# Superjomn/TiPS

Measured on AMD Instinct MI355X. Metric: device-resident fp32 bucket-sum GiB/s (% HBM peak); allreduce GiB/s 1/2/4/8 GPU, higher is better.
Workload: dtype f32

## Files before the change

### tips_amd/csrc/fusion.cc

```cpp
#include <string.h>

#include <algorithm>

#include "rt.h"

namespace tips {
namespace rt {

namespace {

constexpr int64_t kDefaultCopyTile = 8 * 1024;
constexpr size_t kMaxLayouts = 32;
constexpr size_t kMaxTables = 16;
constexpr int kUploadSlots = 4;

int64_t copy_tile_bytes() {
  const int64_t t = env_i64("TIPS_COPY_TILE_BYTES", kDefaultCopyTile);
  return t <= 4096 ? 4096 : t <= 8192 ? 8192 : 16384;
}

int64_t cast_tile_bytes() {
  const int64_t t = env_i64("TIPS_CAST_TILE_BYTES", 4096);
  return t <= 4096 ? 4096 : t <= 8192 ? 8192 : 16384;
}
// ... 264 lines not shown
      const size_t share = std::min<size_t>((size_t)cap, (slow.size() - si + (7 - x)) / (8 - x));
      for (size_t k = 0; k < share; k++) xcd[x].push_back(slow[si++]);
    }
    for (int x = 0; x < 8; x++) {
      const int cap = std::max(0, std::min(R, n - x * R));
      while ((int)xcd[x].size() < cap && si < slow.size()) xcd[x].push_back(slow[si++]);
      while ((int)xcd[x].size() < cap && fi < fast.size()) xcd[x].push_back(fast[fi++]);
    }
    int at = g0;
    for (int x = 0; x < 8; x++)
      for (int j : xcd[x]) order[at++] = j;
  }
  return order;
}

void fill_records(const Layout& L, int mode, const BatchItem* items, const void* base, std::vector<CopySeg>* dst) {
  const int nseg = (int)L.seg_tensor.size();
  const int ntab = tables_of(mode);
  const size_t per = 2 * (size_t)L.ntiles + nseg;
  const int64_t es = tips::dtype_size(L.dtype);
  std::vector<CopySeg>& rec = *dst;
  rec.assign(ntab * per, CopySeg{0, 0, 0, 0});
  for (int k = 0; k < nseg; k++) {
    const int i = L.seg_tensor[k];
    const int64_t b = L.off[i], e = b + L.counts[i] * es;
    const int64_t in = (int64_t)(uintptr_t)items[i].in - b, out = (int64_t)(uintptr_t)items[i].out - b;
    CopySeg* r = rec.data() + 2 * L.ntiles + k;
    if (mode == kSlot || mode == kSlotCast) {
      const int bk = L.bucket[i];
      const int64_t slot = bk < 0 ? 0 : (int64_t)(uintptr_t)base + (int64_t)(bk % 2) * L.threshold - L.buckets[bk].off;
      const int64_t win = (int64_t)(uintptr_t)items[i].in - 2 * b, wout = (int64_t)(uintptr_t)items[i].out - 2 * b;
// ... 4 lines not shown
    } else {
      r[0] = CopySeg{in, (int64_t)(uintptr_t)base, b, e};
    }
  }
  const std::vector<int> order = tile_order(L);
  for (int tb = 0; tb < ntab; tb++) {
    CopySeg* T = rec.data() + tb * per;
    const CopySeg* S = T + 2 * L.ntiles;
    for (int q = 0; q < L.ntiles; q++) {
      const int j = order[q];
      const int first = L.tiles[2 * j], cnt = L.tiles[2 * j + 1];
      T[2 * q] = cnt <= 2 ? S[first] : CopySeg{first, cnt, 0, -1};
      T[2 * q + 1] = cnt == 2 ? S[first + 1] : CopySeg{0, 0, (int64_t)j * L.tile, 0};
    }
  }
}

Table* find_table(State& st, FusionCache& fc, Layout& L, int mode, const BatchItem* items, int n,
                  const void* base) {
  uint64_t h = fnv(fnv(kFnvBasis, (uint64_t)mode), (uint64_t)(uintptr_t)base);
  for (int i = 0; i < n; i++) h = fnv(fnv(h, (uint64_t)(uintptr_t)items[i].in), (uint64_t)(uintptr_t)items[i].out);
  for (Table* t : L.tables) {
    if (t->hash != h || t->mode != mode || t->base != base) continue;
    bool same = true;
    for (int i = 0; i < n && same; i++) same = t->ins[i] == items[i].in && t->outs[i] == items[i].out;
    if (same) {
      t->stamp = ++fc.clock;
      fc.table_hits++;
      if (st.fuse_capturing) t->pinned = true;
      return t;
// ... 6 lines not shown
  }
  Table* t = nullptr;
  size_t unpinned = 0;
  for (const Table* u : L.tables) unpinned += !u->pinned;
  if (unpinned >= kMaxTables) {
    auto lru = L.tables.end();
    for (auto it = L.tables.begin(); it != L.tables.end(); ++it)
      if (!(*it)->pinned && (lru == L.tables.end() || (*it)->stamp < (*lru)->stamp)) lru = it;
    if ((*lru)->mode == mode) {
      t = *lru;
    } else {
      free_table(st, *lru);
      L.tables.erase(lru);
    }
  }
  const int nseg = (int)L.seg_tensor.size();
  const int ntab = tables_of(mode);
  const size_t per = 2 * (size_t)L.ntiles + nseg;
  if (!t) {
    t = new Table();
    if (hipMallocAsync((void**)&t->dev, ntab * per * sizeof(CopySeg), table_stream(st)) != hipSuccess) {
      delete t;
      fail(TIPS_ERR_HIP, "fusion: hipMallocAsync of a segment table failed");
      return nullptr;
    }
    L.tables.push_back(t);
  }
  t->hash = h;
  t->mode = mode;
  t->base = base;
  t->ins.resize(n);
  t->outs.resize(n);
  for (int i = 0; i < n; i++) {
    t->ins[i] = items[i].in;
    t->outs[i] = items[i].out;
  }
  std::vector<CopySeg> rec;
  fill_records(L, mode, items, base, &rec);
  t->stamp = ++fc.clock;
  fc.tables_built++;
  if (upload(st, fc, t->dev, rec.data(), rec.size() * sizeof(CopySeg)) != 0 ||
      (st.fuse_in_call && join(st.fuse_ws, st.fuse_stream, st.ev_fuse_table) != 0)) {
    t->hash = 0;
    t->ins.clear();
    return nullptr;
  }
  return t;
}

int ensure_slots(State& st, FusionCache& fc, int64_t threshold) {
  if (threshold == st.fusion_threshold && st.fusion.p) return 0;
  bool pinned = false;
  for (const Layout* L : fc.layouts) pinned = pinned || L->pinned();
  if (st.fuse_chain_valid) {
    TRY(chain_event(st));
    HIP_TRY(hipEventSynchronize(st.ev_fuse_chain));
// ... 26 lines not shown
}

int open_layout(State& st, FusionCache& fc, const BatchItem* items, int n, int dtype, const LayoutParams& lp,
                hipStream_t ws, Layout** L) {
  if (st.size > 1) {
    HIP_TRY(hipEventRecord(st.ev_start, ws));
    HIP_TRY(hipStreamWaitEvent(st.bucket_stream, st.ev_start, 0));
  }
  std::vector<int64_t> counts((size_t)n);
  for (int i = 0; i < n; i++) counts[i] = items[i].count;
  *L = find_layout(st, fc, counts.data(), n, dtype, lp);
  return 0;
}

struct Records {
  const CopySeg *tiles, *segs;
};
Records records(const Layout& L, const Table& t, int table) {
  const CopySeg* base = t.dev + (size_t)table * (2 * (size_t)L.ntiles + L.seg_tensor.size());
  return {base, base + 2 * L.ntiles};
}

int copy_tiles(const Layout& L, const Table& t, int table, int tile0, int ntiles, hipStream_t s) {
  const Records r = records(L, t, table);
  HIP_TRY(tips::launch_copy_segs(r.tiles, r.segs, tile0, ntiles, L.tile, copy_store_policy(), s));
  return 0;
}

bool pack_merge(const State& st) { return !st.fuse_capturing && env_i64("TIPS_PACK_MERGE", 0) != 0; }

bool pack_signals_ready(State& st, hipStream_t ws) {
  if (st.pack_signals >= 0) return st.pack_signals == 1;
  st.pack_signals = 0;
  if (env_i64("TIPS_PACK_SIGNALS", 1) == 0) return false;
  int can = 0;
  if (hipDeviceGetAttribute(&can, hipDeviceAttributeCanUseStreamWaitValue, st.device) != hipSuccess || !can) {
    (void)hipGetLastError();
    return false;
  }
  bool ok = hipMalloc((void**)&st.pack_counters, tips::kMaxPackGroups * sizeof(unsigned)) == hipSuccess &&
// ... 14 lines not shown

int pack_buckets(State& st, const Layout& L, const Table& t, int table, int b0, int nb, bool signal, uint64_t* values,
                 hipStream_t s) {
  tips::PackGroups g{};
  g.n = nb;
  g.counters = signal ? st.pack_counters : nullptr;
  for (int k = 0; k < nb; k++) {
    g.tile0[k] = L.buckets[b0 + k].tile0;
    g.ntiles[k] = L.buckets[b0 + k].ntiles;
    if (signal) {
      g.done[k] = static_cast<unsigned long long*>(st.pack_done[k]);
      g.sig_value[k] = st.pack_done_value[k] + 1;
    }
  }
  const Records r = records(L, t, table);
  HIP_TRY(tips::launch_copy_segs_groups(r.tiles, r.segs, g, L.tile, copy_store_policy(), s));
  if (signal)
    for (int k = 0; k < nb; k++) values[k] = ++st.pack_done_value[k];
  return 0;
}

int wait_packed(State& st, int k, uint64_t value) {
  HIP_TRY(hipStreamWaitValue64(st.bucket_stream, st.pack_done[k], value, hipStreamWaitValueGte, ~0ull));
  return 0;
}

struct MergedPacks {
  std::function<int(int)> pack;
  std::function<int(int, hipEvent_t)> wait;
};

// ... 258 lines not shown
  if (n <= 0) return 0;
  FusionCache& fc = cache(st);
  const LayoutParams lp = layout_params(true);
  TRY(ensure_slots(st, fc, lp.threshold));
  return in_fusion(st, user, [&](hipStream_t ws) -> int {
    Layout* L = nullptr;
    TRY(open_layout(st, fc, items, n, wire, lp, ws, &L));
    if (!L) return TIPS_ERR_HIP;
    if (L->seg_tensor.empty()) return 0;
    const int64_t es = tips::dtype_size(wire);
    const int B = (int)L->buckets.size();
    Table* t = B ? find_table(st, fc, *L, kSlotCast, items, n, st.fusion.p) : nullptr;
    if (B && !t) return TIPS_ERR_HIP;
    auto cast = [&](int dir, int b) -> int {
      const Records r = records(*L, *t, dir);
      HIP_TRY(tips::launch_cast_segs(r.tiles, r.segs, L->buckets[b].tile0, L->buckets[b].ntiles, L->tile, dir, wire, ws));
      return 0;
    };
    hipStream_t big = st.size > 1 ? st.bucket_stream : ws;
    for (int i : L->direct) {
      TRY(st.cast_scratch.ensure((size_t)(items[i].count * es)));
      HIP_TRY(tips::launch_cast_range(st.cast_scratch.p, items[i].in, items[i].count, 0, wire, big));
      if (st.size > 1) TRY(allreduce_device(st, st.cast_scratch.p, st.cast_scratch.p, items[i].count, wire, big));
      HIP_TRY(tips::launch_cast_range(items[i].out, st.cast_scratch.p, items[i].count, 1, wire, big));
    }
    if (st.size == 1) {
      for (int b = 0; b < B; b++) {
        TRY(cast(0, b));
        TRY(cast(1, b));
      }
      return 0;
// ... 61 lines not shown
  if (dtype != TIPS_FLOAT32)
    return fail(TIPS_ERR_UNSUPPORTED, "tips_fused_allreduce_cast: the tensors must be TIPS_FLOAT32 (got dtype %d)", dtype);
  if (wire_dtype != TIPS_FLOAT16 && wire_dtype != TIPS_BFLOAT16)
    return fail(TIPS_ERR_UNSUPPORTED, "tips_fused_allreduce_cast: the wire type must be TIPS_FLOAT16 or TIPS_BFLOAT16 "
                                      "(got %d)", wire_dtype);
  if (!outs && n > 0) return fail(TIPS_ERR_INVALID_ARG, "bad tensor list");
  return list_collective(ins, counts, n, dtype, wire_dtype, kOutsEach, outs, nullptr, true,
                         [&](State& st, std::vector<BatchItem>& items) {
                           return fused_allreduce_cast(st, items.data(), n, wire_dtype, (hipStream_t)stream);
                         });
}

#ifdef TIPS_DEV
int64_t tips_fusion_tile_table(const int64_t* counts, int n, int dtype, const int64_t* ins, const int64_t* outs,
                               int64_t* records, int64_t cap, int64_t* ntiles, int64_t* tile_bytes) {
  TRY(check_dtype(dtype));
  if (n < 0 || (n > 0 && (!counts || !ins || !outs))) return fail(TIPS_ERR_INVALID_ARG, "bad list");
  for (int i = 0; i < n; i++)
    if (counts[i] < 0) return fail(TIPS_ERR_INVALID_ARG, "negative count %d", i);
  Layout L;
  build_layout(&L, dtype, layout_params(), counts, n);
  std::vector<BatchItem> items((size_t)n);
  for (int i = 0; i < n; i++) items[i] = BatchItem{(const void*)(uintptr_t)ins[i], (void*)(uintptr_t)outs[i], counts[i]};
  std::vector<tips::CopySeg> rec;
  fill_records(L, kCopy, items.data(), nullptr, &rec);
  if (ntiles) *ntiles = L.ntiles;
  if (tile_bytes) *tile_bytes = L.tile;
  if (records) {
    if (cap < (int64_t)rec.size()) return fail(TIPS_ERR_INVALID_ARG, "tips_fusion_tile_table: %zu records, room for %lld", rec.size(), (long long)cap);
    memcpy(records, rec.data(), rec.size() * sizeof(tips::CopySeg));
  }
  return (int64_t)rec.size();
}
#endif

int64_t tips_fused_layout(const int64_t* counts, int n, int dtype, int64_t* offsets) {
  TRY(check_dtype(dtype));
  if (n < 0 || (n > 0 && !counts)) return fail(TIPS_ERR_INVALID_ARG, "bad count list");
  for (int i = 0; i < n; i++)
    if (counts[i] < 0) return fail(TIPS_ERR_INVALID_ARG, "negative count %d", i);
// ... 70 lines not shown
```

### tips_amd/csrc/kernels.h

```cpp
#pragma once

#include <hip/hip_runtime.h>
#include <stdint.h>

#include <vector>

namespace tips {

int dtype_size(int dtype);

hipError_t launch_sum2(void* dst, const void* a, const void* b, int64_t n, int dtype, hipStream_t s);

constexpr int kMaxSrcs = 16;
hipError_t launch_multi_sum(void* dst, const void* const* srcs, int nsrc, int64_t n, int dtype, hipStream_t s);
hipError_t launch_multi_sum_remote(void* dst, const void* const* srcs, int nsrc, int64_t n, int dtype, hipStream_t s);

enum { kOpSum = 0, kOpMax = 1, kOpMin = 2 };
hipError_t launch_reduce2(void* dst, const void* a, const void* b, int64_t n, int dtype, int op, hipStream_t s);
hipError_t launch_multi_reduce(void* dst, const void* const* srcs, int nsrc, int64_t n, int dtype, int op, hipStream_t s);

struct Scale {
  double pre = 1.0, post = 1.0;
  int op = kOpSum;
  bool on() const { return pre != 1.0 || post != 1.0; }
  bool minmax() const { return op != kOpSum; }
  bool plain() const { return !on() && !minmax(); }
};
hipError_t launch_sum2_scaled(void* dst, const void* a, const void* b, int64_t n, int dtype, double pre, double post,
                              unsigned raw, hipStream_t s);
hipError_t launch_multi_sum_scaled(void* dst, const void* const* srcs, int nsrc, int64_t n, int dtype, double pre,
                                   double post, unsigned raw, hipStream_t s);
hipError_t launch_scale_buf(void* dst, const void* src, int64_t n, int dtype, double pre, double post, hipStream_t s);

struct CopySeg {
  int64_t src, dst;
  int64_t begin, end;
};
hipError_t launch_copy_segs(const CopySeg* tiles, const CopySeg* segs, int tile0, int ntiles, int64_t tile_bytes,
                            int pol, hipStream_t s);
int64_t pack_stripe_vecs();
void stripe_slots(int64_t nslots, int64_t C, std::vector<int>* xcd, std::vector<int64_t>* pos);

constexpr int kMaxPackGroups = 8;
struct PackGroups {
  int n;
  int tile0[kMaxPackGroups], ntiles[kMaxPackGroups];
  unsigned blk0[kMaxPackGroups + 1];
  unsigned* counters;
  unsigned long long* done[kMaxPackGroups];
  unsigned long long sig_value[kMaxPackGroups];
};
hipError_t launch_copy_segs_groups(const CopySeg* tiles, const CopySeg* segs, PackGroups g, int64_t tile_bytes, int pol,
                                   hipStream_t s);

hipError_t launch_cast_segs(const CopySeg* tiles, const CopySeg* segs, int tile0, int ntiles, int64_t tile_bytes,
                            int dir, int wire, hipStream_t s);
hipError_t launch_cast_range(void* dst, const void* src, int64_t n, int dir, int wire, hipStream_t s);

hipError_t launch_copy_buf(void* dst, const void* src, int64_t bytes, hipStream_t s);

struct XferSeg {
  const char* src;
  char* dst;
  int64_t bytes;
};
constexpr int kMaxXferSegs = 16;
constexpr int64_t kXferTileBytes = 16 * 1024;
hipError_t launch_xfer(const XferSeg* segs, int nseg, hipStream_t s);

}
```

### tips_amd/csrc/kernels.hip

```cpp
#include <algorithm>
#include <cstdlib>
#include <type_traits>

#include "kernels_device.h"

namespace tips {

int dtype_size(int dtype) {
  switch (dtype) {
    case kF32: return 4;
    case kF64: return 8;
    case kI32: return 4;
    case kI64: return 8;
    case kF16: return 2;
    case kBF16: return 2;
    default: return 0;
  }
}

typedef __attribute__((address_space(1))) u32x4 g_u32x4;
typedef __attribute__((address_space(1))) unsigned g_u32;
typedef __attribute__((address_space(1))) unsigned short g_u16;
typedef __attribute__((address_space(1))) char g_u8;

// ... 39 lines not shown
#pragma unroll
    for (int k = 0; k < 4; k++)
      if (4 * k < len) *reinterpret_cast<g_u32*>(d + 4 * k) = m.w[k];
  } else {
#pragma unroll
    for (int k = 0; k < 8; k++)
      if (2 * k < len) *reinterpret_cast<g_u16*>(d + 2 * k) = m.h[k];
  }
}

template <int U>
struct SegStage {
  CopySeg L[(int)((int64_t)kBlock * 16 * U / 256) + 1];
};

template <int U, int POL>
__device__ __forceinline__ void copy_seg_tile(const CopySeg* __restrict__ tiles, const CopySeg* __restrict__ segs,
                                              int t, CopySeg* L) {
  constexpr int64_t kTileBytes = (int64_t)kBlock * 16 * U;
  constexpr int kMaxSeg = (int)(kTileBytes / 256) + 1;
  const int64_t* tr = reinterpret_cast<const int64_t*>(tiles + 2 * (int64_t)t);
  const int64_t a_src = tr[0], a_dst = tr[1], a_beg = tr[2], a_end = tr[3];
  const int64_t b_src = tr[4], b_dst = tr[5], b_beg = tr[6], b_end = tr[7];
  const int tid = threadIdx.x;
  const bool multi = a_end < 0, two = b_end > 0;
  const int64_t tb = two ? (b_beg & ~(kTileBytes - 1)) : b_beg;
  if (!multi && !two && a_beg <= tb && a_end >= tb + kTileBytes && ((a_src | a_dst) & 15) == 0) {
    __amdgpu_buffer_rsrc_t rs = __builtin_amdgcn_make_buffer_rsrc((void*)(a_src + tb), (short)0, (int)kTileBytes,
                                                                  0x00020000);
    __amdgpu_buffer_rsrc_t rd = __builtin_amdgcn_make_buffer_rsrc((void*)(a_dst + tb), (short)0, (int)kTileBytes,
                                                                  0x00020000);
    u32x4 v[U];
#pragma unroll
    for (int u = 0; u < U; u++) v[u] = __builtin_amdgcn_raw_buffer_load_b128(rs, (u * kBlock + tid) * 16, 0, 2);
#pragma unroll
    for (int u = 0; u < U; u++)
      __builtin_amdgcn_raw_buffer_store_b128(v[u], rd, (u * kBlock + tid) * 16, 0, POL == 0 ? 0 : POL == 1 ? 2 : 16);
    return;
  }
  int cnt = 1;
  if (multi) {
    const int s0 = (int)a_src;
    cnt = min((int)a_dst, kMaxSeg);
    if (cnt <= 0) return;
    if (tid < cnt) L[tid] = segs[s0 + tid];
    __syncthreads();
  }
  int64_t sp[U], dp[U];
  int len[U];
  bool full[U];
  u32x4 x[U];
  Small m[U];
#pragma unroll
  for (int u = 0; u < U; u++) {
// ... 21 lines not shown
    len[u] = (v >= g_beg && left > 0) ? (int)(left < 16 ? left : 16) : 0;
    sp[u] = g_src + v;
    dp[u] = g_dst + v;
    full[u] = len[u] == 16 && ((sp[u] | dp[u]) & 15) == 0;
    if (full[u]) x[u] = __builtin_nontemporal_load(reinterpret_cast<const g_u32x4*>(sp[u]));
    else if (len[u] > 0) small_load(sp[u], dp[u], len[u], m[u]);
  }
#pragma unroll
  for (int u = 0; u < U; u++) {
    if (full[u]) store16_pol<POL>(dp[u], x[u]);
    else if (len[u] > 0) small_store(sp[u], dp[u], len[u], m[u]);
  }
}

template <int U, int POL>
__global__ __launch_bounds__(kBlock) void copy_segs_kernel(const CopySeg* __restrict__ tiles,
                                                          const CopySeg* __restrict__ segs, int tile0, int ntiles,
                                                          int64_t stripe) {
  __shared__ SegStage<U> st;
  const int64_t tt = stripe_tile(blockIdx.x, gridDim.x, stripe);
  if (tt >= ntiles) return;
  copy_seg_tile<U, POL>(tiles, segs, tile0 + (int)tt, st.L);
}


template <int WT>
__device__ __forceinline__ u32x2 narrow4(f32x4 a) {
  if constexpr (WT == kF16) {
    return __builtin_bit_cast(u32x2, __builtin_convertvector(a, f16x4));
  } else {
    const u32x4 x = __builtin_bit_cast(u32x4, a);
    return u32x2{bf16_round_bits(x[0]) | (bf16_round_bits(x[1]) << 16), bf16_round_bits(x[2]) | (bf16_round_bits(x[3]) << 16)};
  }
}

template <int WT>
__device__ __forceinline__ f32x4 widen4(u32x2 v) {
// ... 33 lines not shown
  } else {
    u32x4 x[U];
#pragma unroll
    for (int u = 0; u < U; u++)
      x[u] = __builtin_nontemporal_load(reinterpret_cast<const g_u32x4*>(wire_base + 16 * (int64_t)(u * kBlock + tid)));
#pragma unroll
    for (int u = 0; u < U; u++) reinterpret_cast<u32x4*>(W)[u * kBlock + tid] = x[u];
    __syncthreads();
#pragma unroll
    for (int u = 0; u < 2 * U; u++)
      store16_pol<2>(f32_base + 16 * (int64_t)(u * kBlock + tid), __builtin_bit_cast(u32x4, widen4<WT>(W[u * kBlock + tid])));
  }
}

template <int U, int DIR, int WT, int VAR = 8>
__global__ __launch_bounds__(kBlock) void cast_segs_kernel(const CopySeg* __restrict__ tiles,
                                                          const CopySeg* __restrict__ segs, int tile0, int ntiles) {
  constexpr int64_t kTileBytes = (int64_t)kBlock * 16 * U;
  constexpr int kMaxSeg = (int)(kTileBytes / 256) + 1;
  constexpr int Q = 2 * U;
  __shared__ CopySeg L[kMaxSeg];
  const int64_t tt = xcd_tile(blockIdx.x, gridDim.x);
  if (tt >= ntiles) return;
  const int64_t* tr = reinterpret_cast<const int64_t*>(tiles + 2 * (int64_t)(tile0 + tt));
  const int64_t a_src = tr[0], a_dst = tr[1], a_beg = tr[2], a_end = tr[3];
  const int64_t b_src = tr[4], b_dst = tr[5], b_beg = tr[6], b_end = tr[7];
  const int tid = threadIdx.x;
  const bool multi = a_end < 0, two = b_end > 0;
  const int64_t tb = two ? (b_beg & ~(kTileBytes - 1)) : b_beg;
  if constexpr ((VAR & 8) != 0) {
    __shared__ u32x2 W[kBlock * Q];
    if (!multi && !two && a_beg <= tb && a_end >= tb + kTileBytes && ((a_src | a_dst) & 15) == 0) {
      if constexpr (DIR == 0) cast_tile_staged<U, 0, WT>(a_src + 2 * tb, a_dst + tb, W);
      else cast_tile_staged<U, 1, WT>(a_dst + 2 * tb, a_src + tb, W);
      return;
    }
  }
  int cnt = 1;
  if (multi) {
    cnt = min((int)a_dst, kMaxSeg);
    if (cnt <= 0) return;
    if (tid < cnt) L[tid] = segs[(int)a_src + tid];
    __syncthreads();
  }
  int64_t sp[Q], dp[Q];
  int len[Q];
  bool full[Q];
  u32x2 nv[Q];
  f32x4 wa[Q];
#pragma unroll
  for (int u = 0; u < Q; u++) {
    const int64_t v = tb + (int64_t)u * (kBlock * 8) + (int64_t)tid * 8;
// ... 75 lines not shown
      if constexpr (DIR == 0)
        store8_sc1(wire_side + 8 * q, narrow4<WT>(__builtin_nontemporal_load(reinterpret_cast<const g_f32x4*>(f32_side + 16 * q))));
      else
        store16_pol<2>(f32_side + 16 * q, __builtin_bit_cast(u32x4, widen4<WT>(
                                              __builtin_nontemporal_load(reinterpret_cast<const g_u32x2*>(wire_side + 8 * q)))));
    }
    head = 4 * nq;
  }
  for (int64_t i = head + (int64_t)blockIdx.x * kBlock + threadIdx.x; i < n; i += stride) {
    if constexpr (DIR == 0) static_cast<unsigned short*>(dst)[i] = narrow1<WT>(static_cast<const float*>(src)[i]);
    else static_cast<float*>(dst)[i] = widen1<WT>(static_cast<const unsigned short*>(src)[i]);
  }
}

template <int U, int POL>
__global__ __launch_bounds__(kBlock) void copy_segs_groups_kernel(const CopySeg* __restrict__ tiles,
                                                                 const CopySeg* __restrict__ segs, PackGroups g) {
  __shared__ SegStage<U> st;
  int k = 0;
  while (k + 1 < g.n && blockIdx.x >= g.blk0[k + 1]) k++;
  const unsigned local = blockIdx.x - g.blk0[k], gk = g.blk0[k + 1] - g.blk0[k];
  const int64_t tt = xcd_tile(local, gk);
  if (tt < g.ntiles[k]) copy_seg_tile<U, POL>(tiles, segs, g.tile0[k] + (int)tt, st.L);
  if (g.done[k]) {
    __syncthreads();
    if (threadIdx.x == 0 &&
        __hip_atomic_fetch_add(&g.counters[k], 1u, __ATOMIC_ACQ_REL, __HIP_MEMORY_SCOPE_AGENT) == gk - 1) {
      __hip_atomic_store(&g.counters[k], 0u, __ATOMIC_RELAXED, __HIP_MEMORY_SCOPE_AGENT);
      __hip_atomic_store(g.done[k], g.sig_value[k], __ATOMIC_RELEASE, __HIP_MEMORY_SCOPE_SYSTEM);
    }
  }
}


struct XferList {
  XferSeg s[kMaxXferSegs];
};

// ... 364 lines not shown
  if (nsrc == 1) return launch_multi_sum(dst, srcs, nsrc, n, dtype, s);
  switch (dtype) {
    case kF32: return multi_dispatch<kF32>(dst, srcs, nsrc, n, s, true);
    case kF64: return multi_dispatch<kF64>(dst, srcs, nsrc, n, s, true);
    case kI32: return multi_dispatch<kI32>(dst, srcs, nsrc, n, s, true);
    case kI64: return multi_dispatch<kI64>(dst, srcs, nsrc, n, s, true);
    case kF16: return multi_dispatch<kF16>(dst, srcs, nsrc, n, s, true);
    case kBF16: return multi_dispatch<kBF16>(dst, srcs, nsrc, n, s, true);
    default: return hipErrorInvalidValue;
  }
}

namespace {

template <int U>
hipError_t run_copy_segs_groups(const CopySeg* tiles, const CopySeg* segs, const PackGroups& g, int pol, hipStream_t s) {
  const unsigned grid = g.blk0[g.n];
  switch (pol) {
    case 0: hipLaunchKernelGGL((copy_segs_groups_kernel<U, 0>), dim3(grid), dim3(kBlock), 0, s, tiles, segs, g); break;
    case 1: hipLaunchKernelGGL((copy_segs_groups_kernel<U, 1>), dim3(grid), dim3(kBlock), 0, s, tiles, segs, g); break;
    case 2: hipLaunchKernelGGL((copy_segs_groups_kernel<U, 2>), dim3(grid), dim3(kBlock), 0, s, tiles, segs, g); break;
    default: return hipErrorInvalidValue;
  }
  return hipGetLastError();
}

template <int U>
hipError_t run_copy_segs(const CopySeg* tiles, const CopySeg* segs, int tile0, int ntiles, int pol, hipStream_t s) {
  const int64_t C = pack_stripe_vecs() / ((int64_t)kBlock * U);
  const unsigned grid = (unsigned)stripe_grid(ntiles, C);
  switch (pol) {
    case 0: hipLaunchKernelGGL((copy_segs_kernel<U, 0>), dim3(grid), dim3(kBlock), 0, s, tiles, segs, tile0, ntiles, C); break;
    case 1: hipLaunchKernelGGL((copy_segs_kernel<U, 1>), dim3(grid), dim3(kBlock), 0, s, tiles, segs, tile0, ntiles, C); break;
    case 2: hipLaunchKernelGGL((copy_segs_kernel<U, 2>), dim3(grid), dim3(kBlock), 0, s, tiles, segs, tile0, ntiles, C); break;
    default: return hipErrorInvalidValue;
  }
  return hipGetLastError();
}

}

hipError_t launch_copy_segs(const CopySeg* tiles, const CopySeg* segs, int tile0, int ntiles, int64_t tile_bytes,
                            int pol, hipStream_t s) {
  if (ntiles <= 0) return hipSuccess;
  switch (tile_bytes) {
    case 4096: return run_copy_segs<1>(tiles, segs, tile0, ntiles, pol, s);
    case 8192: return run_copy_segs<2>(tiles, segs, tile0, ntiles, pol, s);
    case 16384: return run_copy_segs<4>(tiles, segs, tile0, ntiles, pol, s);
    default: return hipErrorInvalidValue;
  }
}

hipError_t launch_copy_segs_groups(const CopySeg* tiles, const CopySeg* segs, PackGroups g, int64_t tile_bytes, int pol,
                                   hipStream_t s) {
  if (g.n < 1 || g.n > kMaxPackGroups) return hipErrorInvalidValue;
  for (int k = 0; k < g.n; k++)
    if (g.done[k] && !g.counters) return hipErrorInvalidValue;
  int64_t blk = 0;
  for (int k = 0; k < g.n; k++) {
    if (g.ntiles[k] < 0) return hipErrorInvalidValue;
    g.blk0[k] = (unsigned)blk;
    blk += std::max<int64_t>(8, ((int64_t)g.ntiles[k] + 7) / 8 * 8);
  }
  if (blk > 0x7fffffff) return hipErrorInvalidValue;
  g.blk0[g.n] = (unsigned)blk;
  switch (tile_bytes) {
    case 4096: return run_copy_segs_groups<1>(tiles, segs, g, pol, s);
    case 8192: return run_copy_segs_groups<2>(tiles, segs, g, pol, s);
    case 16384: return run_copy_segs_groups<4>(tiles, segs, g, pol, s);
    default: return hipErrorInvalidValue;
  }
}

namespace {
int cast_lds_bytes(int dir) {
  static const int v[2] = {(int)std::min<long>(65536, std::max<long>(0, getenv("TIPS_CAST_LDS_PACK") ? atol(getenv("TIPS_CAST_LDS_PACK")) : 0)),
                           (int)std::min<long>(65536, std::max<long>(0, getenv("TIPS_CAST_LDS_UNPACK") ? atol(getenv("TIPS_CAST_LDS_UNPACK")) : 0))};
  return v[dir];
}

template <int U, int DIR>
hipError_t run_cast_segs(const CopySeg* tiles, const CopySeg* segs, int tile0, int ntiles, int wire, hipStream_t s) {
  const unsigned grid = (unsigned)std::max<int64_t>(8, ((int64_t)ntiles + 7) / 8 * 8);
  const int lds = cast_lds_bytes(DIR);
  static const int var = getenv("TIPS_CAST_VARIANT") ? atoi(getenv("TIPS_CAST_VARIANT")) : 8;
  if (wire != kF16 && wire != kBF16) return hipErrorInvalidValue;
  auto kern = wire == kF16 ? &cast_segs_kernel<U, DIR, kF16> : &cast_segs_kernel<U, DIR, kBF16>;
  if constexpr (U == 2) {
    if (wire == kF16 && var != 8)
      kern = var == 0   ? &cast_segs_kernel<U, DIR, kF16, 0>
             : var == 1 ? &cast_segs_kernel<U, DIR, kF16, 1>
             : var == 2 ? &cast_segs_kernel<U, DIR, kF16, 2>
             : var == 3 ? &cast_segs_kernel<U, DIR, kF16, 3>
             : var == 4 ? &cast_segs_kernel<U, DIR, kF16, 4>
                        : &cast_segs_kernel<U, DIR, kF16, 5>;
  }
  hipLaunchKernelGGL(kern, dim3(grid), dim3(kBlock), lds, s, tiles, segs, tile0, ntiles);
  return hipGetLastError();
}

template <int DIR>
hipError_t run_cast_range(void* dst, const void* src, int64_t n, int wire, hipStream_t s) {
  const int64_t grid = std::max<int64_t>(1, std::min<int64_t>((n + kBlock - 1) / kBlock, (int64_t)kNumCUs * 16));
  if (wire == kF16) hipLaunchKernelGGL((cast_range_kernel<DIR, kF16>), dim3((unsigned)grid), dim3(kBlock), 0, s, dst, src, n);
  else if (wire == kBF16) hipLaunchKernelGGL((cast_range_kernel<DIR, kBF16>), dim3((unsigned)grid), dim3(kBlock), 0, s, dst, src, n);
  else return hipErrorInvalidValue;
  return hipGetLastError();
}
}

hipError_t launch_cast_segs(const CopySeg* tiles, const CopySeg* segs, int tile0, int ntiles, int64_t tile_bytes,
                            int dir, int wire, hipStream_t s) {
  if (ntiles <= 0) return hipSuccess;
  if (dir != 0 && dir != 1) return hipErrorInvalidValue;
  switch (tile_bytes) {
    case 4096: return dir ? run_cast_segs<1, 1>(tiles, segs, tile0, ntiles, wire, s) : run_cast_segs<1, 0>(tiles, segs, tile0, ntiles, wire, s);
    case 8192: return dir ? run_cast_segs<2, 1>(tiles, segs, tile0, ntiles, wire, s) : run_cast_segs<2, 0>(tiles, segs, tile0, ntiles, wire, s);
    case 16384: return dir ? run_cast_segs<4, 1>(tiles, segs, tile0, ntiles, wire, s) : run_cast_segs<4, 0>(tiles, segs, tile0, ntiles, wire, s);
    default: return hipErrorInvalidValue;
  }
}

hipError_t launch_cast_range(void* dst, const void* src, int64_t n, int dir, int wire, hipStream_t s) {
  if (n <= 0) return hipSuccess;
  return dir ? run_cast_range<1>(dst, src, n, wire, s) : run_cast_range<0>(dst, src, n, wire, s);
}

hipError_t launch_xfer(const XferSeg* segs, int nseg, hipStream_t s) {
  if (nseg < 0 || nseg > kMaxXferSegs) return hipErrorInvalidValue;
  XferList L{};
  int64_t max_tiles = 0;
  int m = 0;
  for (int i = 0; i < nseg; i++) {
// ... 14 lines not shown
```

### tips_amd/csrc/kernels_dev.hip

```cpp
#include <algorithm>

#include "kernels_dev.h"
#include "kernels_device.h"

namespace tips {

template <int DT, int MODE, int UNROLL, bool NTL, bool NTS, int BLOCK>
__global__ __launch_bounds__(BLOCK) void sum2_kernel(u32x4* __restrict__ dst, const u32x4* __restrict__ a,
                                                    const u32x4* __restrict__ b, int64_t nvec, int64_t tail_begin,
                                                    int64_t n) {
  constexpr int64_t kTile = (int64_t)BLOCK * UNROLL;
  const int tid = threadIdx.x;
  int64_t t = (MODE == 2) ? xcd_tile(blockIdx.x, gridDim.x) : (int64_t)blockIdx.x;
  const int64_t tstride = (MODE == 0) ? (int64_t)gridDim.x : 0;
  do {
    const int64_t base = t * kTile + tid;
    if (base + (UNROLL - 1) * BLOCK < nvec) {
      u32x4 x[UNROLL], y[UNROLL];
#pragma unroll
      for (int u = 0; u < UNROLL; u++) x[u] = ld16<NTL>(a + base + u * BLOCK);
#pragma unroll
      for (int u = 0; u < UNROLL; u++) y[u] = ld16<NTL>(b + base + u * BLOCK);
#pragma unroll
      for (int u = 0; u < UNROLL; u++) st16<NTS>(dst + base + u * BLOCK, add16<DT>(x[u], y[u]));
    } else {
#pragma unroll
      for (int u = 0; u < UNROLL; u++) {
        const int64_t i = base + u * BLOCK;
        if (i < nvec) st16<NTS>(dst + i, add16<DT>(ld16<NTL>(a + i), ld16<NTL>(b + i)));
      }
    }
    t += tstride;
  } while (MODE == 0 && t * kTile < nvec);
  if (blockIdx.x == 0 && tail_begin + tid < n) add_elem<DT>(dst, a, b, tail_begin + tid);
}

__global__ __launch_bounds__(256) void sum2_map_kernel(u32x4* __restrict__ dst, const u32x4* __restrict__ a,
                                                       const u32x4* __restrict__ b, int64_t nvec, int64_t tail_begin,
                                                       int64_t n, int64_t stripe) {
  constexpr int64_t kTile = 256;
  const int64_t bx = blockIdx.x, x = bx & 7, j = bx >> 3;
  const int64_t t = stripe == 0 ? bx : (x + 8 * (j / stripe)) * stripe + j % stripe;
  const int64_t first = t * kTile;
  if (first < nvec) {
    const int rec = (int)(((nvec - first) < kTile ? (nvec - first) : kTile) * 16);
    __amdgpu_buffer_rsrc_t ra = __builtin_amdgcn_make_buffer_rsrc((void*)(a + first), (short)0, rec, 0x00020000);
    __amdgpu_buffer_rsrc_t rb = __builtin_amdgcn_make_buffer_rsrc((void*)(b + first), (short)0, rec, 0x00020000);
    __amdgpu_buffer_rsrc_t rd = __builtin_amdgcn_make_buffer_rsrc((void*)(dst + first), (short)0, rec, 0x00020000);
    const u32x4 xv = __builtin_amdgcn_raw_buffer_load_b128(ra, (int)threadIdx.x * 16, 0, 2);
// ... 290 lines not shown

template <int DT>
hipError_t sum2_dispatch(void* dst, const void* a, const void* b, int64_t n, int mode, int unroll, int nt, int blocks,
                         int threads, hipStream_t s) {
  if (!(aligned16(dst) && aligned16(a) && aligned16(b))) return launch_sum2(dst, a, b, n, DT, s);
  if (mode == 5) {
    if constexpr (DT == kF32) {
      if (threads == 256 && (unroll == 1 || unroll == 2 || unroll == 4 || unroll == 8)) {
        const int64_t nvec = n / 4;
        hipLaunchKernelGGL(sum2_stream_kernel, dim3((unsigned)(kNumCUs * unroll)), dim3(256), 0, s, (u32x4*)dst,
                           (const u32x4*)a, (const u32x4*)b, nvec, nvec * 4, n);
        return hipGetLastError();
      }
    }
    return hipErrorInvalidValue;
  }
  if (mode == 6) {
    if constexpr (DT == kF32) {
      const int64_t nvec = n / 4, T = (nvec + 255) / 256;
      const int64_t stripe = (int64_t)unroll * 1024 / 4096;
      if (unroll < 0 || (unroll > 0 && stripe < 1)) return hipErrorInvalidValue;
      const int64_t grid = stripe == 0 ? std::max<int64_t>(1, T) : ((T + stripe - 1) / stripe + 7) / 8 * 8 * stripe;
      hipLaunchKernelGGL(sum2_map_kernel, dim3((unsigned)grid), dim3(256), 0, s, (u32x4*)dst, (const u32x4*)a,
                         (const u32x4*)b, nvec, nvec * 4, n, stripe);
      return hipGetLastError();
    }
    return hipErrorInvalidValue;
  }
  if (mode == 4) {
    if constexpr (DT == kF32) {
// ... 327 lines not shown
```

Before: 6296.

## Add precomputed per-tile descriptors for fast-path whole-tile copies and casts

Builds a compact per-tile descriptor table (absolute src/dst addresses) alongside the existing segment records. Kernels check it first and take the single-segment buffer copy or cast path without reading and decoding the 64-byte tile records. Descriptors are loaded into scalar registers, and a look-ahead touch warms the descriptor cache for later tiles. The change also adds a dev-only bound copy kernel mode. The cost is a larger device table, extra upload bytes, and one more dependent load on the slow path.

```diff
diff --git a/tips_amd/csrc/fusion.cc b/tips_amd/csrc/fusion.cc
--- a/tips_amd/csrc/fusion.cc
+++ b/tips_amd/csrc/fusion.cc
@@ -302,7 +302,8 @@
   return order;
 }
 
-void fill_records(const Layout& L, int mode, const BatchItem* items, const void* base, std::vector<CopySeg>* dst) {
+void fill_records(const Layout& L, int mode, const BatchItem* items, const void* base, std::vector<CopySeg>* dst,
+                  std::vector<tips::TileDesc>* descs) {
   const int nseg = (int)L.seg_tensor.size();
   const int ntab = tables_of(mode);
   const size_t per = 2 * (size_t)L.ntiles + nseg;
@@ -337,6 +338,24 @@
       T[2 * q + 1] = cnt == 2 ? S[first + 1] : CopySeg{0, 0, (int64_t)j * L.tile, 0};
     }
   }
+  descs->assign((size_t)ntab * L.ntiles, tips::TileDesc{tips::kDescRecords, 0});
+  for (int tb = 0; tb < ntab; tb++) {
+    const CopySeg* S = rec.data() + tb * per + 2 * L.ntiles;
+    const int64_t ks = mode == kSlotCast && tb == 0 ? 2 : 1, kd = mode == kSlotCast && tb == 1 ? 2 : 1;
+    for (int q = 0; q < L.ntiles; q++) {
+      const int j = order[q];
+      const int64_t v = (int64_t)j * L.tile;
+      if (L.tiles[2 * j + 1] != 1) continue;
+      const CopySeg& g = S[L.tiles[2 * j]];
+      if (g.begin <= v && g.end >= v + L.tile && ((g.src | g.dst) & 15) == 0)
+        (*descs)[(size_t)tb * L.ntiles + q] = tips::TileDesc{g.src + ks * v, g.dst + kd * v};
+    }
+  }
+}
+
+size_t table_bytes(const Layout& L, int mode) {
+  const size_t per = 2 * (size_t)L.ntiles + L.seg_tensor.size();
+  return tables_of(mode) * (per * sizeof(CopySeg) + (size_t)L.ntiles * sizeof(tips::TileDesc));
 }
 
 Table* find_table(State& st, FusionCache& fc, Layout& L, int mode, const BatchItem* items, int n,
@@ -373,12 +392,9 @@
       L.tables.erase(lru);
     }
   }
-  const int nseg = (int)L.seg_tensor.size();
-  const int ntab = tables_of(mode);
-  const size_t per = 2 * (size_t)L.ntiles + nseg;
   if (!t) {
     t = new Table();
-    if (hipMallocAsync((void**)&t->dev, ntab * per * sizeof(CopySeg), table_stream(st)) != hipSuccess) {
+    if (hipMallocAsync((void**)&t->dev, table_bytes(L, mode), table_stream(st)) != hipSuccess) {
       delete t;
       fail(TIPS_ERR_HIP, "fusion: hipMallocAsync of a segment table failed");
       return nullptr;
@@ -395,10 +411,14 @@
     t->outs[i] = items[i].out;
   }
   std::vector<CopySeg> rec;
-  fill_records(L, mode, items, base, &rec);
+  std::vector<tips::TileDesc> descs;
+  fill_records(L, mode, items, base, &rec, &descs);
+  const size_t nrec = rec.size();
+  rec.resize(nrec + (descs.size() + 1) / 2);
+  memcpy(static_cast<void*>(rec.data() + nrec), descs.data(), descs.size() * sizeof(tips::TileDesc));
   t->stamp = ++fc.clock;
   fc.tables_built++;
-  if (upload(st, fc, t->dev, rec.data(), rec.size() * sizeof(CopySeg)) != 0 ||
+  if (upload(st, fc, t->dev, rec.data(), table_bytes(L, mode)) != 0 ||
       (st.fuse_in_call && join(st.fuse_ws, st.fuse_stream, st.ev_fuse_table) != 0)) {
     t->hash = 0;
     t->ins.clear();
@@ -455,16 +475,19 @@
 }
 
 struct Records {
+  const tips::TileDesc* desc;
   const CopySeg *tiles, *segs;
 };
 Records records(const Layout& L, const Table& t, int table) {
-  const CopySeg* base = t.dev + (size_t)table * (2 * (size_t)L.ntiles + L.seg_tensor.size());
-  return {base, base + 2 * L.ntiles};
+  const size_t per = 2 * (size_t)L.ntiles + L.seg_tensor.size();
+  const CopySeg* base = t.dev + (size_t)table * per;
+  const tips::TileDesc* desc = reinterpret_cast<const tips::TileDesc*>(t.dev + (size_t)tables_of(t.mode) * per);
+  return {desc + (size_t)table * L.ntiles, base, base + 2 * L.ntiles};
 }
 
 int copy_tiles(const Layout& L, const Table& t, int table, int tile0, int ntiles, hipStream_t s) {
   const Records r = records(L, t, table);
-  HIP_TRY(tips::launch_copy_segs(r.tiles, r.segs, tile0, ntiles, L.tile, copy_store_policy(), s));
+  HIP_TRY(tips::launch_copy_segs(r.desc, r.tiles, r.segs, tile0, ntiles, L.tile, copy_store_policy(), s));
   return 0;
 }
 
@@ -509,7 +532,7 @@
     }
   }
   const Records r = records(L, t, table);
-  HIP_TRY(tips::launch_copy_segs_groups(r.tiles, r.segs, g, L.tile, copy_store_policy(), s));
+  HIP_TRY(tips::launch_copy_segs_groups(r.desc, r.tiles, r.segs, g, L.tile, copy_store_policy(), s));
   if (signal)
     for (int k = 0; k < nb; k++) values[k] = ++st.pack_done_value[k];
   return 0;
@@ -798,7 +821,7 @@
     if (B && !t) return TIPS_ERR_HIP;
     auto cast = [&](int dir, int b) -> int {
       const Records r = records(*L, *t, dir);
-      HIP_TRY(tips::launch_cast_segs(r.tiles, r.segs, L->buckets[b].tile0, L->buckets[b].ntiles, L->tile, dir, wire, ws));
+      HIP_TRY(tips::launch_cast_segs(r.desc, r.tiles, r.segs, L->buckets[b].tile0, L->buckets[b].ntiles, L->tile, dir, wire, ws));
       return 0;
     };
     hipStream_t big = st.size > 1 ? st.bucket_stream : ws;
@@ -890,16 +913,27 @@
 #ifdef TIPS_DEV
 int64_t tips_fusion_tile_table(const int64_t* counts, int n, int dtype, const int64_t* ins, const int64_t* outs,
                                int64_t* records, int64_t cap, int64_t* ntiles, int64_t* tile_bytes) {
+  constexpr uintptr_t kTestSlotBase = (uintptr_t)1 << 41;
   TRY(check_dtype(dtype));
   if (n < 0 || (n > 0 && (!counts || !ins || !outs))) return fail(TIPS_ERR_INVALID_ARG, "bad list");
   for (int i = 0; i < n; i++)
     if (counts[i] < 0) return fail(TIPS_ERR_INVALID_ARG, "negative count %d", i);
+  const int64_t with_descs = env_i64("TIPS_TILE_TABLE_DESCS", 0);
+  const bool cast = with_descs == 2;
+  if (cast && dtype != TIPS_FLOAT16 && dtype != TIPS_BFLOAT16)
+    return fail(TIPS_ERR_INVALID_ARG, "tips_fusion_tile_table: a cast table's dtype is the wire type (got %d)", dtype);
   Layout L;
-  build_layout(&L, dtype, layout_params(), counts, n);
+  build_layout(&L, dtype, layout_params(cast), counts, n);
   std::vector<BatchItem> items((size_t)n);
   for (int i = 0; i < n; i++) items[i] = BatchItem{(const void*)(uintptr_t)ins[i], (void*)(uintptr_t)outs[i], counts[i]};
   std::vector<tips::CopySeg> rec;
-  fill_records(L, kCopy, items.data(), nullptr, &rec);
+  std::vector<tips::TileDesc> descs;
+  fill_records(L, cast ? kSlotCast : kCopy, items.data(), cast ? (const void*)kTestSlotBase : nullptr, &rec, &descs);
+  if (with_descs != 0) {
+    const size_t nrec = rec.size();
+    rec.resize(nrec + (descs.size() + 1) / 2, tips::CopySeg{0, 0, 0, 0});
+    memcpy(static_cast<void*>(rec.data() + nrec), descs.data(), descs.size() * sizeof(tips::TileDesc));
+  }
   if (ntiles) *ntiles = L.ntiles;
   if (tile_bytes) *tile_bytes = L.tile;
   if (records) {
diff --git a/tips_amd/csrc/kernels.h b/tips_amd/csrc/kernels.h
--- a/tips_amd/csrc/kernels.h
+++ b/tips_amd/csrc/kernels.h
@@ -36,8 +36,12 @@
   int64_t src, dst;
   int64_t begin, end;
 };
-hipError_t launch_copy_segs(const CopySeg* tiles, const CopySeg* segs, int tile0, int ntiles, int64_t tile_bytes,
-                            int pol, hipStream_t s);
+struct TileDesc {
+  int64_t src, dst;
+};
+constexpr int64_t kDescRecords = 1;
+hipError_t launch_copy_segs(const TileDesc* desc, const CopySeg* tiles, const CopySeg* segs, int tile0, int ntiles,
+                            int64_t tile_bytes, int pol, hipStream_t s);
 int64_t pack_stripe_vecs();
 void stripe_slots(int64_t nslots, int64_t C, std::vector<int>* xcd, std::vector<int64_t>* pos);
 
@@ -50,11 +54,11 @@
   unsigned long long* done[kMaxPackGroups];
   unsigned long long sig_value[kMaxPackGroups];
 };
-hipError_t launch_copy_segs_groups(const CopySeg* tiles, const CopySeg* segs, PackGroups g, int64_t tile_bytes, int pol,
-                                   hipStream_t s);
+hipError_t launch_copy_segs_groups(const TileDesc* desc, const CopySeg* tiles, const CopySeg* segs, PackGroups g,
+                                   int64_t tile_bytes, int pol, hipStream_t s);
 
-hipError_t launch_cast_segs(const CopySeg* tiles, const CopySeg* segs, int tile0, int ntiles, int64_t tile_bytes,
-                            int dir, int wire, hipStream_t s);
+hipError_t launch_cast_segs(const TileDesc* desc, const CopySeg* tiles, const CopySeg* segs, int tile0, int ntiles,
+                            int64_t tile_bytes, int dir, int wire, hipStream_t s);
 hipError_t launch_cast_range(void* dst, const void* src, int64_t n, int dir, int wire, hipStream_t s);
 
 hipError_t launch_copy_buf(void* dst, const void* src, int64_t bytes, hipStream_t s);
diff --git a/tips_amd/csrc/kernels.hip b/tips_amd/csrc/kernels.hip
--- a/tips_amd/csrc/kernels.hip
+++ b/tips_amd/csrc/kernels.hip
@@ -77,30 +77,42 @@
   CopySeg L[(int)((int64_t)kBlock * 16 * U / 256) + 1];
 };
 
+__device__ __forceinline__ TileDesc load_desc(const TileDesc* __restrict__ desc, int64_t t) {
+  const int64_t* p = reinterpret_cast<const int64_t*>(desc + t);
+  TileDesc d{p[0], p[1]};
+  asm volatile("" : "+s"(d.src), "+s"(d.dst));
+  return d;
+}
+
+constexpr int kAheadSlots = 32 * 8;
+__device__ __forceinline__ int64_t touch_ahead(const TileDesc* __restrict__ desc, int tile0, int ntiles, int64_t tt) {
+  const int64_t la = tt + kAheadSlots < ntiles ? tt + kAheadSlots : (int64_t)ntiles - 1;
+  return reinterpret_cast<const int64_t*>(desc + tile0 + la)[0];
+}
+__device__ __forceinline__ void touch_done(int64_t touched) { asm volatile("" ::"s"(touched)); }
+
 template <int U, int POL>
-__device__ __forceinline__ void copy_seg_tile(const CopySeg* __restrict__ tiles, const CopySeg* __restrict__ segs,
-                                              int t, CopySeg* L) {
+__device__ __forceinline__ void copy_seg_tile(TileDesc d, const CopySeg* __restrict__ tiles,
+                                              const CopySeg* __restrict__ segs, int t, CopySeg* L) {
   constexpr int64_t kTileBytes = (int64_t)kBlock * 16 * U;
   constexpr int kMaxSeg = (int)(kTileBytes / 256) + 1;
+  const int tid = threadIdx.x;
+  if ((d.src & 15) == 0) {
+    __amdgpu_buffer_rsrc_t rs = __builtin_amdgcn_make_buffer_rsrc((void*)d.src, (short)0, (int)kTileBytes, 0x00020000);
+    __amdgpu_buffer_rsrc_t rd = __builtin_amdgcn_make_buffer_rsrc((void*)d.dst, (short)0, (int)kTileBytes, 0x00020000);
+    u32x4 v[U];
+#pragma unroll
+    for (int u = 0; u < U; u++) v[u] = __builtin_amdgcn_raw_buffer_load_b128(rs, (u * kBlock + tid) * 16, 0, 2);
+#pragma unroll
+    for (int u = 0; u < U; u++)
+      __builtin_amdgcn_raw_buffer_store_b128(v[u], rd, (u * kBlock + tid) * 16, 0, POL == 0 ? 0 : POL == 1 ? 2 : 16);
+    return;
+  }
   const int64_t* tr = reinterpret_cast<const int64_t*>(tiles + 2 * (int64_t)t);
   const int64_t a_src = tr[0], a_dst = tr[1], a_beg = tr[2], a_end = tr[3];
   const int64_t b_src = tr[4], b_dst = tr[5], b_beg = tr[6], b_end = tr[7];
-  const int tid = threadIdx.x;
   const bool multi = a_end < 0, two = b_end > 0;
   const int64_t tb = two ? (b_beg & ~(kTileBytes - 1)) : b_beg;
-  if (!multi && !two && a_beg <= tb && a_end >= tb + kTileBytes && ((a_src | a_dst) & 15) == 0) {
-    __amdgpu_buffer_rsrc_t rs = __builtin_amdgcn_make_buffer_rsrc((void*)(a_src + tb), (short)0, (int)kTileBytes,
-                                                                  0x00020000);
-    __amdgpu_buffer_rsrc_t rd = __builtin_amdgcn_make_buffer_rsrc((void*)(a_dst + tb), (short)0, (int)kTileBytes,
-                                                                  0x00020000);
-    u32x4 v[U];
-#pragma unroll
-    for (int u = 0; u < U; u++) v[u] = __builtin_amdgcn_raw_buffer_load_b128(rs, (u * kBlock + tid) * 16, 0, 2);
-#pragma unroll
-    for (int u = 0; u < U; u++)
-      __builtin_amdgcn_raw_buffer_store_b128(v[u], rd, (u * kBlock + tid) * 16, 0, POL == 0 ? 0 : POL == 1 ? 2 : 16);
-    return;
-  }
   int cnt = 1;
   if (multi) {
     const int s0 = (int)a_src;
@@ -152,13 +164,18 @@
 }
 
 template <int U, int POL>
-__global__ __launch_bounds__(kBlock) void copy_segs_kernel(const CopySeg* __restrict__ tiles,
+__global__ __launch_bounds__(kBlock) void copy_segs_kernel(const TileDesc* __restrict__ desc,
+                                                          const CopySeg* __restrict__ tiles,
                                                           const CopySeg* __restrict__ segs, int tile0, int ntiles,
                                                           int64_t stripe) {
   __shared__ SegStage<U> st;
+  asm volatile("" ::"s"(tile0), "s"(ntiles));
   const int64_t tt = stripe_tile(blockIdx.x, gridDim.x, stripe);
+  const TileDesc d = load_desc(desc, tile0 + (tt < ntiles ? tt : (int64_t)ntiles - 1));
   if (tt >= ntiles) return;
-  copy_seg_tile<U, POL>(tiles, segs, tile0 + (int)tt, st.L);
+  const int64_t touched = touch_ahead(desc, tile0, ntiles, tt);
+  copy_seg_tile<U, POL>(d, tiles, segs, tile0 + (int)tt, st.L);
+  touch_done(touched);
 }
 
 
@@ -222,28 +239,31 @@
 }
 
 template <int U, int DIR, int WT, int VAR = 8>
-__global__ __launch_bounds__(kBlock) void cast_segs_kernel(const CopySeg* __restrict__ tiles,
+__global__ __launch_bounds__(kBlock) void cast_segs_kernel(const TileDesc* __restrict__ desc,
+                                                          const CopySeg* __restrict__ tiles,
                                                           const CopySeg* __restrict__ segs, int tile0, int ntiles) {
   constexpr int64_t kTileBytes = (int64_t)kBlock * 16 * U;
   constexpr int kMaxSeg = (int)(kTileBytes / 256) + 1;
   constexpr int Q = 2 * U;
   __shared__ CopySeg L[kMaxSeg];
+  asm volatile("" ::"s"(tile0), "s"(ntiles));
   const int64_t tt = xcd_tile(blockIdx.x, gridDim.x);
+  const TileDesc d = load_desc(desc, tile0 + (tt < ntiles ? tt : (int64_t)ntiles - 1));
   if (tt >= ntiles) return;
+  if constexpr ((VAR & 8) != 0) {
+    __shared__ u32x2 W[kBlock * Q];
+    if ((d.src & 15) == 0) {
+      if constexpr (DIR == 0) cast_tile_staged<U, 0, WT>(d.src, d.dst, W);
+      else cast_tile_staged<U, 1, WT>(d.dst, d.src, W);
+      return;
+    }
+  }
   const int64_t* tr = reinterpret_cast<const int64_t*>(tiles + 2 * (int64_t)(tile0 + tt));
   const int64_t a_src = tr[0], a_dst = tr[1], a_beg = tr[2], a_end = tr[3];
   const int64_t b_src = tr[4], b_dst = tr[5], b_beg = tr[6], b_end = tr[7];
   const int tid = threadIdx.x;
   const bool multi = a_end < 0, two = b_end > 0;
   const int64_t tb = two ? (b_beg & ~(kTileBytes - 1)) : b_beg;
-  if constexpr ((VAR & 8) != 0) {
-    __shared__ u32x2 W[kBlock * Q];
-    if (!multi && !two && a_beg <= tb && a_end >= tb + kTileBytes && ((a_src | a_dst) & 15) == 0) {
-      if constexpr (DIR == 0) cast_tile_staged<U, 0, WT>(a_src + 2 * tb, a_dst + tb, W);
-      else cast_tile_staged<U, 1, WT>(a_dst + 2 * tb, a_src + tb, W);
-      return;
-    }
-  }
   int cnt = 1;
   if (multi) {
     cnt = min((int)a_dst, kMaxSeg);
@@ -349,14 +369,18 @@
 }
 
 template <int U, int POL>
-__global__ __launch_bounds__(kBlock) void copy_segs_groups_kernel(const CopySeg* __restrict__ tiles,
+__global__ __launch_bounds__(kBlock) void copy_segs_groups_kernel(const TileDesc* __restrict__ desc,
+                                                                 const CopySeg* __restrict__ tiles,
                                                                  const CopySeg* __restrict__ segs, PackGroups g) {
   __shared__ SegStage<U> st;
   int k = 0;
   while (k + 1 < g.n && blockIdx.x >= g.blk0[k + 1]) k++;
   const unsigned local = blockIdx.x - g.blk0[k], gk = g.blk0[k + 1] - g.blk0[k];
   const int64_t tt = xcd_tile(local, gk);
-  if (tt < g.ntiles[k]) copy_seg_tile<U, POL>(tiles, segs, g.tile0[k] + (int)tt, st.L);
+  if (tt < g.ntiles[k]) {
+    const int t = g.tile0[k] + (int)tt;
+    copy_seg_tile<U, POL>(load_desc(desc, t), tiles, segs, t, st.L);
+  }
   if (g.done[k]) {
     __syncthreads();
     if (threadIdx.x == 0 &&
@@ -751,25 +775,27 @@
 namespace {
 
 template <int U>
-hipError_t run_copy_segs_groups(const CopySeg* tiles, const CopySeg* segs, const PackGroups& g, int pol, hipStream_t s) {
+hipError_t run_copy_segs_groups(const TileDesc* desc, const CopySeg* tiles, const CopySeg* segs, const PackGroups& g,
+                                int pol, hipStream_t s) {
   const unsigned grid = g.blk0[g.n];
   switch (pol) {
-    case 0: hipLaunchKernelGGL((copy_segs_groups_kernel<U, 0>), dim3(grid), dim3(kBlock), 0, s, tiles, segs, g); break;
-    case 1: hipLaunchKernelGGL((copy_segs_groups_kernel<U, 1>), dim3(grid), dim3(kBlock), 0, s, tiles, segs, g); break;
-    case 2: hipLaunchKernelGGL((copy_segs_groups_kernel<U, 2>), dim3(grid), dim3(kBlock), 0, s, tiles, segs, g); break;
+    case 0: hipLaunchKernelGGL((copy_segs_groups_kernel<U, 0>), dim3(grid), dim3(kBlock), 0, s, desc, tiles, segs, g); break;
+    case 1: hipLaunchKernelGGL((copy_segs_groups_kernel<U, 1>), dim3(grid), dim3(kBlock), 0, s, desc, tiles, segs, g); break;
+    case 2: hipLaunchKernelGGL((copy_segs_groups_kernel<U, 2>), dim3(grid), dim3(kBlock), 0, s, desc, tiles, segs, g); break;
     default: return hipErrorInvalidValue;
   }
   return hipGetLastError();
 }
 
 template <int U>
-hipError_t run_copy_segs(const CopySeg* tiles, const CopySeg* segs, int tile0, int ntiles, int pol, hipStream_t s) {
+hipError_t run_copy_segs(const TileDesc* desc, const CopySeg* tiles, const CopySeg* segs, int tile0, int ntiles, int pol,
+                         hipStream_t s) {
   const int64_t C = pack_stripe_vecs() / ((int64_t)kBlock * U);
   const unsigned grid = (unsigned)stripe_grid(ntiles, C);
   switch (pol) {
-    case 0: hipLaunchKernelGGL((copy_segs_kernel<U, 0>), dim3(grid), dim3(kBlock), 0, s, tiles, segs, tile0, ntiles, C); break;
-    case 1: hipLaunchKernelGGL((copy_segs_kernel<U, 1>), dim3(grid), dim3(kBlock), 0, s, tiles, segs, tile0, ntiles, C); break;
-    case 2: hipLaunchKernelGGL((copy_segs_kernel<U, 2>), dim3(grid), dim3(kBlock), 0, s, tiles, segs, tile0, ntiles, C); break;
+    case 0: hipLaunchKernelGGL((copy_segs_kernel<U, 0>), dim3(grid), dim3(kBlock), 0, s, desc, tiles, segs, tile0, ntiles, C); break;
+    case 1: hipLaunchKernelGGL((copy_segs_kernel<U, 1>), dim3(grid), dim3(kBlock), 0, s, desc, tiles, segs, tile0, ntiles, C); break;
+    case 2: hipLaunchKernelGGL((copy_segs_kernel<U, 2>), dim3(grid), dim3(kBlock), 0, s, desc, tiles, segs, tile0, ntiles, C); break;
     default: return hipErrorInvalidValue;
   }
   return hipGetLastError();
@@ -777,19 +803,19 @@
 
 }
 
-hipError_t launch_copy_segs(const CopySeg* tiles, const CopySeg* segs, int tile0, int ntiles, int64_t tile_bytes,
-                            int pol, hipStream_t s) {
+hipError_t launch_copy_segs(const TileDesc* desc, const CopySeg* tiles, const CopySeg* segs, int tile0, int ntiles,
+                            int64_t tile_bytes, int pol, hipStream_t s) {
   if (ntiles <= 0) return hipSuccess;
   switch (tile_bytes) {
-    case 4096: return run_copy_segs<1>(tiles, segs, tile0, ntiles, pol, s);
-    case 8192: return run_copy_segs<2>(tiles, segs, tile0, ntiles, pol, s);
-    case 16384: return run_copy_segs<4>(tiles, segs, tile0, ntiles, pol, s);
-    default: return hipErrorInvalidValue;
-  }
-}
-
-hipError_t launch_copy_segs_groups(const CopySeg* tiles, const CopySeg* segs, PackGroups g, int64_t tile_bytes, int pol,
-                                   hipStream_t s) {
+    case 4096: return run_copy_segs<1>(desc, tiles, segs, tile0, ntiles, pol, s);
+    case 8192: return run_copy_segs<2>(desc, tiles, segs, tile0, ntiles, pol, s);
+    case 16384: return run_copy_segs<4>(desc, tiles, segs, tile0, ntiles, pol, s);
+    default: return hipErrorInvalidValue;
+  }
+}
+
+hipError_t launch_copy_segs_groups(const TileDesc* desc, const CopySeg* tiles, const CopySeg* segs, PackGroups g,
+                                   int64_t tile_bytes, int pol, hipStream_t s) {
   if (g.n < 1 || g.n > kMaxPackGroups) return hipErrorInvalidValue;
   for (int k = 0; k < g.n; k++)
     if (g.done[k] && !g.counters) return hipErrorInvalidValue;
@@ -802,9 +828,9 @@
   if (blk > 0x7fffffff) return hipErrorInvalidValue;
   g.blk0[g.n] = (unsigned)blk;
   switch (tile_bytes) {
-    case 4096: return run_copy_segs_groups<1>(tiles, segs, g, pol, s);
-    case 8192: return run_copy_segs_groups<2>(tiles, segs, g, pol, s);
-    case 16384: return run_copy_segs_groups<4>(tiles, segs, g, pol, s);
+    case 4096: return run_copy_segs_groups<1>(desc, tiles, segs, g, pol, s);
+    case 8192: return run_copy_segs_groups<2>(desc, tiles, segs, g, pol, s);
+    case 16384: return run_copy_segs_groups<4>(desc, tiles, segs, g, pol, s);
     default: return hipErrorInvalidValue;
   }
 }
@@ -817,7 +843,8 @@
 }
 
 template <int U, int DIR>
-hipError_t run_cast_segs(const CopySeg* tiles, const CopySeg* segs, int tile0, int ntiles, int wire, hipStream_t s) {
+hipError_t run_cast_segs(const TileDesc* desc, const CopySeg* tiles, const CopySeg* segs, int tile0, int ntiles, int wire,
+                         hipStream_t s) {
   const unsigned grid = (unsigned)std::max<int64_t>(8, ((int64_t)ntiles + 7) / 8 * 8);
   const int lds = cast_lds_bytes(DIR);
   static const int var = getenv("TIPS_CAST_VARIANT") ? atoi(getenv("TIPS_CAST_VARIANT")) : 8;
@@ -832,7 +859,7 @@
              : var == 4 ? &cast_segs_kernel<U, DIR, kF16, 4>
                         : &cast_segs_kernel<U, DIR, kF16, 5>;
   }
-  hipLaunchKernelGGL(kern, dim3(grid), dim3(kBlock), lds, s, tiles, segs, tile0, ntiles);
+  hipLaunchKernelGGL(kern, dim3(grid), dim3(kBlock), lds, s, desc, tiles, segs, tile0, ntiles);
   return hipGetLastError();
 }
 
@@ -846,14 +873,14 @@
 }
 }
 
-hipError_t launch_cast_segs(const CopySeg* tiles, const CopySeg* segs, int tile0, int ntiles, int64_t tile_bytes,
-                            int dir, int wire, hipStream_t s) {
+hipError_t launch_cast_segs(const TileDesc* desc, const CopySeg* tiles, const CopySeg* segs, int tile0, int ntiles,
+                            int64_t tile_bytes, int dir, int wire, hipStream_t s) {
   if (ntiles <= 0) return hipSuccess;
   if (dir != 0 && dir != 1) return hipErrorInvalidValue;
   switch (tile_bytes) {
-    case 4096: return dir ? run_cast_segs<1, 1>(tiles, segs, tile0, ntiles, wire, s) : run_cast_segs<1, 0>(tiles, segs, tile0, ntiles, wire, s);
-    case 8192: return dir ? run_cast_segs<2, 1>(tiles, segs, tile0, ntiles, wire, s) : run_cast_segs<2, 0>(tiles, segs, tile0, ntiles, wire, s);
-    case 16384: return dir ? run_cast_segs<4, 1>(tiles, segs, tile0, ntiles, wire, s) : run_cast_segs<4, 0>(tiles, segs, tile0, ntiles, wire, s);
+    case 4096: return dir ? run_cast_segs<1, 1>(desc, tiles, segs, tile0, ntiles, wire, s) : run_cast_segs<1, 0>(desc, tiles, segs, tile0, ntiles, wire, s);
+    case 8192: return dir ? run_cast_segs<2, 1>(desc, tiles, segs, tile0, ntiles, wire, s) : run_cast_segs<2, 0>(desc, tiles, segs, tile0, ntiles, wire, s);
+    case 16384: return dir ? run_cast_segs<4, 1>(desc, tiles, segs, tile0, ntiles, wire, s) : run_cast_segs<4, 0>(desc, tiles, segs, tile0, ntiles, wire, s);
     default: return hipErrorInvalidValue;
   }
 }
diff --git a/tips_amd/csrc/kernels_dev.hip b/tips_amd/csrc/kernels_dev.hip
--- a/tips_amd/csrc/kernels_dev.hip
+++ b/tips_amd/csrc/kernels_dev.hip
@@ -33,6 +33,23 @@
     t += tstride;
   } while (MODE == 0 && t * kTile < nvec);
   if (blockIdx.x == 0 && tail_begin + tid < n) add_elem<DT>(dst, a, b, tail_begin + tid);
+}
+
+template <int U>
+__global__ __launch_bounds__(kBlock) void copy_bound_kernel(char* __restrict__ dst, const char* __restrict__ src,
+                                                           int64_t bytes) {
+  constexpr int64_t kTileBytes = (int64_t)kBlock * 16 * U;
+  const int64_t tb = xcd_tile(blockIdx.x, gridDim.x) * kTileBytes;
+  if (tb >= bytes) return;
+  const int rec = (int)(bytes - tb < kTileBytes ? bytes - tb : kTileBytes);
+  __amdgpu_buffer_rsrc_t rs = __builtin_amdgcn_make_buffer_rsrc((void*)(src + tb), (short)0, rec, 0x00020000);
+  __amdgpu_buffer_rsrc_t rd = __builtin_amdgcn_make_buffer_rsrc((void*)(dst + tb), (short)0, rec, 0x00020000);
+  const int tid = threadIdx.x;
+  u32x4 v[U];
+#pragma unroll
+  for (int u = 0; u < U; u++) v[u] = __builtin_amdgcn_raw_buffer_load_b128(rs, (u * kBlock + tid) * 16, 0, 2);
+#pragma unroll
+  for (int u = 0; u < U; u++) __builtin_amdgcn_raw_buffer_store_b128(v[u], rd, (u * kBlock + tid) * 16, 0, 16);
 }
 
 __global__ __launch_bounds__(256) void sum2_map_kernel(u32x4* __restrict__ dst, const u32x4* __restrict__ a,
@@ -353,6 +370,16 @@
       }
     }
     return hipErrorInvalidValue;
+  }
+  if (mode == 7) {
+    const int64_t bytes = n * (int64_t)dtype_size(DT) / 16 * 16;
+    if (threads != kBlock || (unroll != 1 && unroll != 2 && unroll != 4)) return hipErrorInvalidValue;
+    const int64_t tiles = (bytes + (int64_t)kBlock * 16 * unroll - 1) / ((int64_t)kBlock * 16 * unroll);
+    const dim3 grid((unsigned)std::max<int64_t>(8, (tiles + 7) / 8 * 8));
+    if (unroll == 1) hipLaunchKernelGGL((copy_bound_kernel<1>), grid, dim3(kBlock), 0, s, (char*)dst, (const char*)a, bytes);
+    else if (unroll == 2) hipLaunchKernelGGL((copy_bound_kernel<2>), grid, dim3(kBlock), 0, s, (char*)dst, (const char*)a, bytes);
+    else hipLaunchKernelGGL((copy_bound_kernel<4>), grid, dim3(kBlock), 0, s, (char*)dst, (const char*)a, bytes);
+    return hipGetLastError();
   }
   if (mode == 6) {
     if constexpr (DT == kF32) {
```

New measurement: 6328, median of 2. Within noise of the previous version (+0.5%).
